# microsoft/SpareNet

Measured on AMD Instinct MI355X. Metric: point-pairs/sec (CD+EMD) + depthmaps/sec, B=32 N=16384, higher is better.
Workload: dtype f32

## Files before the change

### sparenet_amd/csrc/p2i.hip

```cpp
#include <cmath>
#include <cstring>

#include "block_scan.hpp"
#include "common.hpp"
#include "wave_dpp.hpp"

namespace {

__device__ __forceinline__ int clampi(int v, int lo, int hi) {
  return v < lo ? lo : (v > hi ? hi : v);
}

struct Box {
  int min_x, max_x, min_y, max_y;
};
__device__ __forceinline__ Box box_of(float py, float px, int h, int w, float radius) {
  Box b;
  b.min_x = clampi((int)floorf(px - radius), 0, w - 1);
  b.max_x = clampi((int)ceilf(px + radius), 0, w - 1);
  b.min_y = clampi((int)floorf(py - radius), 0, h - 1);
  b.max_y = clampi((int)ceilf(py + radius), 0, h - 1);
  return b;
}

__device__ __forceinline__ float cos_weight_inv(float r, double inv_radius) {
  const double y = ((double)r * inv_radius - 0.5) * M_PI;
  const double y2 = y * y;
  double p = -3.868170170630684e-23;
  p = __builtin_fma(p, y2, 1.9572941063391263e-20);
  p = __builtin_fma(p, y2, -8.22063524662433e-18);
  p = __builtin_fma(p, y2, 2.8114572543455206e-15);
  p = __builtin_fma(p, y2, -7.647163731819816e-13);
  p = __builtin_fma(p, y2, 1.6059043836821613e-10);
  p = __builtin_fma(p, y2, -2.505210838544172e-08);
  p = __builtin_fma(p, y2, 2.7557319223985893e-06);
  p = __builtin_fma(p, y2, -0.0001984126984126984);
  p = __builtin_fma(p, y2, 0.008333333333333333);
  p = __builtin_fma(p, y2, -0.16666666666666666);
  p = __builtin_fma(p, y2, 1.0);
  return (float)(0.5 - 0.5 * (y * p));
}
__device__ __forceinline__ float cos_weight(float r, float radius) {
  return cos_weight_inv(r, 1.0 / (double)radius);
}

__device__ __forceinline__ float sq2(float dx, float dy) {
#pragma clang fp contract(off)
  return dx * dx + dy * dy;
}

__device__ __forceinline__ float radius_of(float dx, float dy) {
#pragma clang fp contract(off)
  return __builtin_sqrtf(dx * dx + dy * dy);
}

__device__ __forceinline__ float one_zero(float v) { return v == 0.f ? 0.f : v; }

__global__ __launch_bounds__(256) void p2i_max_init_kernel(const float *__restrict__ background,
                                                           unsigned long long *__restrict__ img,
                                                           long total) {
  for (long e = (long)blockIdx.x * blockDim.x + threadIdx.x; e < total;
       e += (long)gridDim.x * blockDim.x)
    img[e] = ((unsigned long long)sn::ordered_key(one_zero(background[e])) << 32) | 0xFFFFFFFFull;
}

__device__ __forceinline__ long xcd_point_group(int lpp, int npoints, int channels, int batch) {
  const int gpb = 256 / lpp;
  const long chunk = ((long)npoints + batch - 1) / batch * channels;
  const int bpc = (int)((chunk + gpb - 1) / gpb);
  const int g = blockIdx.x, xcd = g & 7, r = g >> 3;
  const int cidx = (r / bpc) * 8 + xcd;
  if (cidx >= batch) return -1;
  const long local = (long)(r % bpc) * gpb + threadIdx.x / lpp;
  if (local >= chunk) return -1;
  const long gid = (long)cidx * chunk + local;
  return gid < (long)npoints * channels ? gid : -1;
}
inline long xcd_point_blocks(int lpp, int npoints, int channels, int batch) {
  const int gpb = 256 / lpp;
  const long chunk = ((long)npoints + batch - 1) / batch * channels;
  const long bpc = (chunk + gpb - 1) / gpb;
  return bpc * 8 * ((batch + 7) / 8);
}

struct SplatHit {
  unsigned pix;
  float r, f;
  unsigned low;
};

__device__ __forceinline__ float max_sq_inside(float radius) {
#pragma clang fp contract(off)
  float s = radius * radius;
  while (__builtin_sqrtf(s) > radius) s = __uint_as_float(__float_as_uint(s) - 1u);
  for (;;) {
    const float t = __uint_as_float(__float_as_uint(s) + 1u);
    if (!(__builtin_sqrtf(t) <= radius)) break;
    s = t;
  }
  return s;
}

__device__ __forceinline__ void splat_exact(const SplatHit &hh, unsigned long long *img,
                                            float radius) {
  const float v = one_zero(hh.f * cos_weight(__builtin_sqrtf(hh.r), radius));
  atomicMax(img + hh.pix, ((unsigned long long)sn::ordered_key(v) << 32) | hh.low);
}

template <int LPP>
__global__ __launch_bounds__(256) void p2i_max_splat_kernel(
    const float *__restrict__ points, const float *__restrict__ feat,
    const int *__restrict__ batch_inds, unsigned long long *__restrict__ img, int npoints,
    int channels, int batch, int h, int w, float radius) {
  constexpr int kQ = 128;
  __shared__ SplatHit queue[4][kQ];
  const int wave = threadIdx.x >> 6, lane = threadIdx.x & 63;
  SplatHit *q = queue[wave];
  const long gid = xcd_point_group(LPP, npoints, channels, batch);
  const int l = threadIdx.x % LPP;
  bool alive = gid >= 0;
  int x = 0, y = 0, min_y = 0, max_y = -1, max_x = -1;
  float px = 0.f, py = 0.f, f = 0.f;
  unsigned low = 0, plane = 0;
  if (alive) {
    const int c = (int)(gid % channels);
    const int pid = (int)((gid / channels) % npoints);
    const int b = batch_inds[pid];
    if (b < 0 || b >= batch) {
      alive = false;
    } else {
      py = points[pid * 2 + 0];
      px = points[pid * 2 + 1];
      f = feat[gid];
      const Box bx = box_of(py, px, h, w, radius);
      x = bx.min_x + l;
      y = min_y = bx.min_y;
      max_y = bx.max_y;
      max_x = bx.max_x;
      low = 0xFFFFFFFEu - (unsigned)pid;
      plane = (unsigned)(((size_t)b * channels + c) * h * w);
      alive = x <= max_x;
    }
  }
  const float rev_scale = 0.5f / radius;
  const float s_max = max_sq_inside(radius);
  int qn = 0;
  constexpr int kRows = 8;
  while (__any(alive)) {
    float s2[kRows];
    unsigned pix[kRows], cur[kRows];
    bool in[kRows];
    const float dx = x - px;
#pragma unroll
    for (int i = 0; i < kRows; ++i) {
      const int yy = y + i;
      s2[i] = sq2(dx, yy - py);
      in[i] = alive && yy <= max_y && s2[i] <= s_max;
      pix[i] = in[i] ? plane + (unsigned)yy * w + x : plane;
    }
#pragma unroll
    for (int i = 0; i < kRows; ++i)
      cur[i] = (unsigned)(__hip_atomic_load(img + pix[i], __ATOMIC_RELAXED,
                                            __HIP_MEMORY_SCOPE_AGENT) >> 32);
#pragma unroll
    for (int i = 0; i < kRows; ++i) {
      bool pass = false;
      if (in[i]) {
        const float ra = __builtin_amdgcn_sqrtf(s2[i]);
        const float wq = __builtin_amdgcn_cosf(ra * rev_scale) * 0.5f + 0.5f;
        const float ub = f >= 0.f ? f * (wq + 2e-5f) : f * __builtin_fmaxf(wq - 2e-5f, 0.f);
        pass = !(sn::ordered_key(one_zero(ub)) < cur[i]);
      }
      const unsigned long long m = __ballot(pass);
      if (m) {
        if (pass)
          q[qn + __builtin_amdgcn_mbcnt_hi((unsigned)(m >> 32), __builtin_amdgcn_mbcnt_lo((unsigned)m, 0u))] =
              SplatHit{pix[i], s2[i], f, low};
        qn += __popcll(m);
        __builtin_amdgcn_fence(__ATOMIC_RELEASE, "wavefront");
        if (qn >= 64) {
          __builtin_amdgcn_fence(__ATOMIC_ACQUIRE, "wavefront");
          qn -= 64;
          splat_exact(q[qn + lane], img, radius);
          __builtin_amdgcn_fence(__ATOMIC_ACQ_REL, "wavefront");
        }
      }
    }
    if (alive) {
      y += kRows;
      if (y > max_y) {
        y = min_y;
        x += LPP;
        alive = x <= max_x;
      }
    }
  }
  __builtin_amdgcn_fence(__ATOMIC_ACQUIRE, "wavefront");
  if (lane < qn) splat_exact(q[lane], img, radius);
}

constexpr int kCell = 8;
constexpr int kMaxRadii = 4;

struct RadiiArg {
  float radius[kMaxRadii], s_max[kMaxRadii], rev_scale[kMaxRadii], inv_r2[kMaxRadii];
  float s_max_all;
  int halo;
};

__device__ __forceinline__ int cell_of_point(float py, float px, int h, int w, int cells_x,
                                             int cells_y) {
  if (!(__builtin_fabsf(py) < 1e9f) || !(__builtin_fabsf(px) < 1e9f)) return -1;
  const int cy = clampi((int)floorf(py) / kCell, 0, cells_y - 1);
  const int cx = clampi((int)floorf(px) / kCell, 0, cells_x - 1);
  (void)h;
  (void)w;
  return cy * cells_x + cx;
}

__global__ __launch_bounds__(256) void p2i_bin_count_kernel(
    const float *__restrict__ points, const int *__restrict__ batch_inds, int *__restrict__ offs,
    int npoints, int batch, int h, int w, int cells_x, int cells_y, const unsigned *__restrict__ need) {
  if (*need == 0u) return;
  for (int pid = blockIdx.x * blockDim.x + threadIdx.x; pid < npoints;
       pid += gridDim.x * blockDim.x) {
    const int b = batch_inds[pid];
    if (b < 0 || b >= batch) continue;
    const int c = cell_of_point(points[pid * 2 + 0], points[pid * 2 + 1], h, w, cells_x, cells_y);
    if (c >= 0) atomicAdd(&offs[b * cells_y * cells_x + c], 1);
  }
}

__global__ __launch_bounds__(1024) void p2i_bin_scan_kernel(const int *__restrict__ counts,
                                                            int *__restrict__ offs_out,
                                                            int cells_per_image,
                                                            const unsigned *__restrict__ need) {
  __shared__ alignas(16) sn::BlockScan<1024> scan;
  if (*need == 0u) return;
  const int tid = threadIdx.x, b = blockIdx.x;
  int before = 0;
  for (long i = tid; i < (long)b * cells_per_image; i += 1024) before += counts[i];
  for (int m = 1; m < 64; m <<= 1) before += __shfl_xor(before, m);
  if ((tid & 63) == 0) scan.wsum[tid >> 6] = before;
  __syncthreads();
  int t = 0;
  if (tid == 0)
    for (int w = 0; w < 16; ++w) t += scan.wsum[w];
  scan.reset(t);
  const int *c = counts + (size_t)b * cells_per_image;
  int *o = offs_out + (size_t)b * cells_per_image;
  for (int base = 0; base < cells_per_image; base += 1024) {
    const int i = base + tid;
    scan.chunk(i < cells_per_image ? c[i] : 0, [&](int start) {
      if (i < cells_per_image) o[i] = start;
    });
  }
}

__global__ __launch_bounds__(256) void p2i_bin_scatter_kernel(
    const float *__restrict__ points, const float *__restrict__ feat,
    const int *__restrict__ batch_inds, int *__restrict__ offs, float4 *__restrict__ srec,
    unsigned *__restrict__ fmax_bits, int npoints, int channels, int batch, int h, int w, int cells_x,
    int cells_y, const unsigned *__restrict__ need) {
  if (*need == 0u) return;
  float fm = 0.f;
  for (int pid = blockIdx.x * blockDim.x + threadIdx.x; pid < npoints;
       pid += gridDim.x * blockDim.x) {
    const int b = batch_inds[pid];
    if (b < 0 || b >= batch) continue;
    const float py = points[pid * 2 + 0], px = points[pid * 2 + 1];
    const int c = cell_of_point(py, px, h, w, cells_x, cells_y);
    if (c < 0) continue;
    const int pos = atomicAdd(&offs[b * cells_y * cells_x + c], 1);
    srec[pos] = make_float4(py, px, channels == 1 ? feat[pid] : 0.f, __int_as_float(pid));
    for (int ch = 0; ch < channels; ++ch) fm = __builtin_fmaxf(fm, __builtin_fabsf(feat[(size_t)pid * channels + ch]));
  }
  for (int m = 1; m < 64; m <<= 1) fm = __builtin_fmaxf(fm, __shfl_xor(fm, m));
  if ((threadIdx.x & 63) == 0 && __float_as_uint(fm) > *reinterpret_cast<volatile unsigned *>(fmax_bits))
    atomicMax(fmax_bits, __float_as_uint(fm));
}

constexpr int kGroupCells = 8192;
__global__ __launch_bounds__(1024) void p2i_bin_grouped_kernel(
    const float *__restrict__ points, const float *__restrict__ feat,
    const int *__restrict__ batch_inds, int *__restrict__ offs, float4 *__restrict__ srec,
    unsigned *__restrict__ fmax_bits, unsigned *__restrict__ need, int ppi, int channels, int h, int w,
    int cells_x, int cells_y) {
  __shared__ int cnt[kGroupCells];
  __shared__ alignas(16) sn::BlockScan<1024> scan;
  __shared__ int bad;
  const int tid = threadIdx.x, b = blockIdx.x;
  const int cpi = cells_x * cells_y;
  const long base = (long)b * ppi;
  for (int i = tid; i < cpi; i += 1024) cnt[i] = 0;
  if (tid == 0) bad = 0;
  __syncthreads();
  bool wrong = false;
  for (int i = tid; i < ppi; i += 1024) {
    const long pid = base + i;
    const int c = cell_of_point(points[pid * 2 + 0], points[pid * 2 + 1], h, w, cells_x, cells_y);
    wrong |= batch_inds[pid] != b || c < 0;
    if (c >= 0) atomicAdd(&cnt[c], 1);
  }
  if (wrong) bad = 1;
  __syncthreads();
  if (bad) {
    if (tid == 0) atomicOr(need, 1u);
    return;
  }
  scan.reset((int)base);
  for (int c0 = 0; c0 < cpi; c0 += 1024) {
    const int i = c0 + tid;
    scan.chunk(i < cpi ? cnt[i] : 0, [&](int start) {
      if (i < cpi) cnt[i] = start;
    });
  }
  float fm = 0.f;
  for (int i = tid; i < ppi; i += 1024) {
    const long pid = base + i;
    const float py = points[pid * 2 + 0], px = points[pid * 2 + 1];
    const int c = cell_of_point(py, px, h, w, cells_x, cells_y);
    const int pos = atomicAdd(&cnt[c], 1);
    srec[pos] = make_float4(py, px, channels == 1 ? feat[pid] : 0.f, __int_as_float((int)pid));
    for (int ch = 0; ch < channels; ++ch) fm = __builtin_fmaxf(fm, __builtin_fabsf(feat[(size_t)pid * channels + ch]));
  }
  __syncthreads();
  for (int i = tid; i < cpi; i += 1024) offs[(long)b * cpi + i] = cnt[i];
  for (int m = 1; m < 64; m <<= 1) fm = __builtin_fmaxf(fm, __shfl_xor(fm, m));
  if ((tid & 63) == 0 && __float_as_uint(fm) > *reinterpret_cast<volatile unsigned *>(fmax_bits))
    atomicMax(fmax_bits, __float_as_uint(fm));
}

#ifdef SN_P2I_DIAG
__device__ unsigned long long g_gather_diag[8];
#define GDIAG(...) __VA_ARGS__
#else
#define GDIAG(...)
#endif

__device__ __forceinline__ float weight32(float u) {
  float p = __builtin_fmaf(u, -0.0102886269f, 0.114825197f);
  p = __builtin_fmaf(u, p, -0.666184545f);
  p = __builtin_fmaf(u, p, 2.02902055f);
  p = __builtin_fmaf(u, p, -2.46737266f);
  return __builtin_fmaf(u, p, 0.999999583f);
}
constexpr float kWeightErr = 1.5e-6f;
__device__ __forceinline__ float weight32_plus(float u, float e) {
  float p = __builtin_fmaf(u, -0.0102886269f, 0.114825197f);
  p = __builtin_fmaf(u, p, -0.666184545f);
  p = __builtin_fmaf(u, p, 2.02902055f);
  p = __builtin_fmaf(u, p, -2.46737266f);
  return __builtin_fmaf(u, p, 0.999999583f + e);
}

__device__ __forceinline__ float slope32(float u) {
  float p = __builtin_fmaf(u, -0.00193834002f, 0.0257028304f);
  p = __builtin_fmaf(u, p, -0.190524563f);
  p = __builtin_fmaf(u, p, 0.811689675f);
  p = __builtin_fmaf(u, p, -1.64492953f);
  return __builtin_fmaf(u, p, 0.99999994f);
}

__global__ void p2i_series_kernel(const float *__restrict__ u, int n, float *__restrict__ w,
                                  float *__restrict__ sl) {
  const int i = blockIdx.x * blockDim.x + threadIdx.x;
  if (i < n) {
    w[i] = weight32(u[i]);
    sl[i] = slope32(u[i]);
  }
}

template <int NR, bool C1>
__global__ __launch_bounds__(256, 6) void p2i_gather_max_kernel(
    const float *__restrict__ feat, const float *__restrict__ background,
    const float4 *__restrict__ srec, const int *__restrict__ offs, const unsigned *__restrict__ fmax_bits,
    int channels, int batch, int h, int w, int cells_x, int cells_y, RadiiArg ra,
    float *__restrict__ out, int *__restrict__ out_ids, long obstride, long orstride) {
  const int wave = __builtin_amdgcn_readfirstlane((int)(threadIdx.x >> 6)), lane = threadIdx.x & 63;
  long tile = (long)blockIdx.x * 4 + wave;
  const long tiles = (long)batch * channels * cells_y * cells_x;
  if (tile >= tiles) return;
  const int cx = (int)(tile % cells_x); tile /= cells_x;
  const int cy = (int)(tile % cells_y); tile /= cells_y;
  const int c = (int)(tile % channels);
  const int b = (int)(tile / channels);
  const int x = cx * kCell + (lane & 7), y = cy * kCell + (lane >> 3);
  const bool valid = x < w && y < h;
  const unsigned long long valid_mask = __builtin_amdgcn_ballot_w64(valid);
  const size_t plane = ((size_t)b * channels + c) * h * w;
  const float fx = (float)x, fy = (float)y;
  const float eps = __uint_as_float(*fmax_bits) * kWeightErr, band = 2.f * eps;
  constexpr unsigned kBg = 0xFFFFFFFFu;
  const float bg = valid && background ? background[plane + (size_t)y * w + x] : 0.f;
  float b1[NR], b2[NR], b3[NR];
  float low1[NR];
  unsigned j1[NR], j2[NR];
#pragma unroll
  for (int k = 0; k < NR; ++k) {
    b1[k] = bg;
    low1[k] = bg - band;
    j1[k] = kBg;
    b2[k] = b3[k] = -3.0e38f;
    j2[k] = kBg;
  }
  const float tx0 = (float)(cx * kCell), tx1 = tx0 + (kCell - 1), ty0 = (float)(cy * kCell),
              ty1 = ty0 + (kCell - 1);
  float tile_min[NR];
  GDIAG(int dg_batches = 0, dg_cand = 0, dg_surv = 0, dg_pairs = 0, dg_upd = 0, dg_amb = 0, dg_walk = 0, dg_rings = 0;)
  bool dirty[NR];
  auto refresh_tile_min = [&]() {
#pragma unroll
    for (int k = 0; k < NR; ++k) {
      if (!dirty[k]) continue;
      dirty[k] = false;
      tile_min[k] = sn::wave_min_f32(valid ? b1[k] : 3.0e38f);
    }
  };
#pragma unroll
  for (int k = 0; k < NR; ++k) dirty[k] = true;
  refresh_tile_min();

  const int cell_base = b * cells_y * cells_x;
  auto row_range = [&](int step, int part, int &beg, int &end) -> bool {
    const int dyc = (step + 1) >> 1;
    const int cyy = cy + ((step & 1) ? -dyc : dyc);
    if (cyy < 0 || cyy >= cells_y) return false;
    const float gy = (float)((dyc > 1 ? dyc - 1 : 0) * kCell);
    const float rem = ra.s_max_all * 1.0001f - gy * gy;
    if (rem < 0.f) return false;
    int reach = (int)(__builtin_sqrtf(rem) * (1.0f / kCell)) + 1;
    reach = reach < ra.halo ? reach : ra.halo;
    const int c_lo = cx - reach > 0 ? cx - reach : 0;
    const int c_hi = cx + reach < cells_x - 1 ? cx + reach : cells_x - 1;
    const int p_lo = step == 0 ? (part == 0 ? cx : (part == 1 ? c_lo : cx + 1)) : c_lo;
    const int p_hi = step == 0 ? (part == 0 ? cx : (part == 1 ? cx - 1 : c_hi)) : c_hi;
    if (p_lo > p_hi) return false;
    const int first_cell = cell_base + cyy * cells_x + p_lo;
    beg = first_cell > 0 ? offs[first_cell - 1] : 0;
    end = offs[cell_base + cyy * cells_x + p_hi];
    return beg < end;
  };

  auto ring_range = [&](int ring, int rstep, int part, int &beg, int &end) -> bool {
    const int dyc = (rstep + 1) >> 1;
    const int cyy = cy + ((rstep & 1) ? -dyc : dyc);
    if (cyy < 0 || cyy >= cells_y) return false;
    const float gy = (float)((dyc > 1 ? dyc - 1 : 0) * kCell);
    const float rem = ra.s_max_all * 1.0001f - gy * gy;
    if (rem < 0.f) return false;
    int p_lo, p_hi;
    if (dyc == ring) {
      if (part != 0) return false;
      int reach = (int)(__builtin_sqrtf(rem) * (1.0f / kCell)) + 1;
      reach = reach < ring ? reach : ring;
      p_lo = cx - reach > 0 ? cx - reach : 0;
      p_hi = cx + reach < cells_x - 1 ? cx + reach : cells_x - 1;
    } else {
      const float gx = (float)((ring - 1) * kCell);
      if (gx * gx > rem) return false;
      p_lo = p_hi = part == 0 ? cx - ring : cx + ring;
      if (p_lo < 0 || p_lo >= cells_x) return false;
    }
    const int first_cell = cell_base + cyy * cells_x + p_lo;
    beg = first_cell > 0 ? offs[first_cell - 1] : 0;
    end = offs[cell_base + cyy * cells_x + p_hi];
    return beg < end;
  };
  const float fmaxv = __uint_as_float(*fmax_bits);
  for (int ring = 0; ring <= ra.halo; ++ring) {
    if (ring >= 2) {
      const float g = (float)((ring - 1) * kCell);
      const float g2 = g * g * 0.99999f;
      bool live = false;
#pragma unroll
      for (int k = 0; k < NR; ++k) {
        const float ub = fmaxv * weight32_plus(__builtin_fminf(g2 * ra.inv_r2[k], 1.0f), 4e-6f);
        live = live || (g2 <= ra.s_max[k] && tile_min[k] <= ub + band);
      }
      GDIAG(dg_rings += live ? 0 : 1;)
      if (!live) break;
    }
   for (int rstep = 0; rstep <= 2 * ring; ++rstep) {
    for (int part = 0; part < 2; ++part) {
      int beg, end;
      if (!ring_range(ring, rstep, part, beg, end)) continue;
      float4 rec_next = make_float4(0.f, 0.f, 0.f, 0.f);
      if (beg + lane < end) rec_next = srec[beg + lane];
      for (int base = beg; base < end; base += 64) {
        const int j = base + lane;
        const float4 rec = rec_next;
        if (j + 64 < end) rec_next = srec[j + 64];
        float cpy = 0.f, cpx = 0.f, cf = 0.f;
        if (j < end) {
          cpy = rec.x;
          cpx = rec.y;
          cf = C1 ? rec.z : feat[(size_t)__float_as_int(rec.w) * channels + c];
        }
        unsigned long long keep[NR];
        {
          const float ddx = __builtin_fmaxf(__builtin_fmaxf(tx0 - cpx, cpx - tx1), 0.f);
          const float ddy = __builtin_fmaxf(__builtin_fmaxf(ty0 - cpy, cpy - ty1), 0.f);
          const float smin = (ddx * ddx + ddy * ddy) * 0.99999f;
          unsigned long long m_end;
          float cfp;
          asm("v_cmp_lt_i32_e64 %0, %1, %2" : "=s"(m_end) : "v"(j), "s"(end));
          asm("v_max_f32 %0, %1, %2" : "=v"(cfp) : "v"(cf), "v"(0.f));
#pragma unroll
          for (int k = 0; k < NR; ++k) {
            float u;
            asm("v_min_f32 %0, %1, %2" : "=v"(u) : "v"(smin * ra.inv_r2[k]), "v"(1.0f));
            const float ub = cfp * weight32_plus(u, 4e-6f);
            unsigned long long m_r, m_v;
            asm("v_cmp_ge_f32_e64 %0, %1, %2" : "=s"(m_r) : "s"(ra.s_max[k]), "v"(smin));
            asm("v_cmp_le_f32_e64 %0, %1, %2" : "=s"(m_v) : "s"(tile_min[k]), "v"(ub + band));
            keep[k] = m_end & m_r & m_v;
          }
        }
        unsigned long long todo = keep[0];
#pragma unroll
        for (int k = 1; k < NR; ++k) todo |= keep[k];
        GDIAG(dg_batches++; dg_cand += (end - base < 64 ? end - base : 64); dg_surv += __popcll(todo);)
        while (todo) {
          const int i = __builtin_ctzll(todo);
          todo &= todo - 1;
          const float py = __int_as_float(__builtin_amdgcn_readlane(__float_as_int(cpy), i));
          const float px = __int_as_float(__builtin_amdgcn_readlane(__float_as_int(cpx), i));
          const float f = __int_as_float(__builtin_amdgcn_readlane(__float_as_int(cf), i));
          const float dx = fx - px, dy = fy - py;
          const float s2 = sq2(dx, dy);
          const unsigned pos = (unsigned)(base + i);
#pragma unroll
          for (int k = 0; k < NR; ++k) {
            if (!((keep[k] >> i) & 1ull)) continue;
            const float a = f * weight32(s2 * ra.inv_r2[k]);
            unsigned long long m_in, m_ge;
            asm("v_cmp_ge_f32_e64 %0, %1, %2" : "=s"(m_in) : "s"(ra.s_max[k]), "v"(s2));
            asm("v_cmp_ge_f32_e64 %0, %1, %2" : "=s"(m_ge) : "v"(a), "v"(low1[k]));
            const unsigned long long pass = m_in & m_ge & valid_mask;
            GDIAG(dg_pairs += __popcll(m_in & valid_mask); dg_upd += __popcll(pass);)
            if (pass != 0ull) {
              dirty[k] = true;
              float ae, t, t2, n1, n2, n3;
              unsigned long long first, second;
              unsigned posv = pos, e2, nj1, nj2;
              const float far = -__builtin_inff();
              asm("v_cndmask_b32_e64 %0, %1, %2, %3" : "=v"(ae) : "v"(far), "v"(a), "s"(pass));
              asm("v_cmp_gt_f32_e64 %0, %1, %2" : "=s"(first) : "v"(ae), "v"(b1[k]));
              asm("v_cmp_gt_f32_e64 %0, %1, %2" : "=s"(second) : "v"(ae), "v"(b2[k]));
              asm("v_min_f32 %0, %1, %2" : "=v"(t) : "v"(b1[k]), "v"(ae));
              asm("v_max_f32 %0, %1, %2" : "=v"(n1) : "v"(b1[k]), "v"(ae));
              asm("v_min_f32 %0, %1, %2" : "=v"(t2) : "v"(b2[k]), "v"(t));
              asm("v_max_f32 %0, %1, %2" : "=v"(n2) : "v"(b2[k]), "v"(t));
              asm("v_max_f32 %0, %1, %2" : "=v"(n3) : "v"(b3[k]), "v"(t2));
              asm("v_cndmask_b32_e64 %0, %1, %2, %3" : "=v"(e2) : "v"(j2[k]), "v"(posv), "s"(second));
              asm("v_cndmask_b32_e64 %0, %1, %2, %3" : "=v"(nj2) : "v"(e2), "v"(j1[k]), "s"(first));
              asm("v_cndmask_b32_e64 %0, %1, %2, %3" : "=v"(nj1) : "v"(j1[k]), "v"(posv), "s"(first));
              j2[k] = nj2;
              j1[k] = nj1;
              b1[k] = n1;
              b2[k] = n2;
              b3[k] = n3;
              low1[k] = n1 - band;
            }
          }
        }
        refresh_tile_min();
      }
    }
   }
  }

  auto exact_of = [&](unsigned pos, double inv_radius, float s_max, float &v, unsigned &low) {
    const float4 rec = srec[pos];
    const int pid = __float_as_int(rec.w);
    const float f = C1 ? rec.z : feat[(size_t)pid * channels + c];
    const float s2 = sq2(fx - rec.y, fy - rec.x);
    (void)s_max;
    v = f * cos_weight_inv(__builtin_sqrtf(s2), inv_radius);
    low = 0xFFFFFFFEu - (unsigned)pid;
  };
  const size_t oplane = (size_t)b * obstride + (size_t)c * h * w;
#pragma unroll
  for (int k = 0; k < NR; ++k) {
    float best_v = bg;
    unsigned best_low = kBg;
    const double inv_rd = 1.0 / (double)ra.radius[k];
    const bool walk = valid && b3[k] >= b1[k] - band;
    const bool amb = valid && !walk && b2[k] >= b1[k] - band;
    GDIAG(dg_amb += __popcll(__ballot(amb)); dg_walk += __popcll(__ballot(walk));)
    if (valid && !walk) {
      auto consider = [&](unsigned pos) {
        if (pos == kBg) return;
        float v;
        unsigned low;
        exact_of(pos, inv_rd, ra.s_max[k], v, low);
        if (v > best_v || (v == best_v && best_low != kBg && low > best_low)) {
          best_v = v;
          best_low = low;
        }
      };
      consider(j1[k]);
      if (amb) consider(j2[k]);
    }
    if (__any(walk)) {
      for (int step = 0; step <= 2 * ra.halo; ++step) {
        const int nparts = step == 0 ? 3 : 1;
        for (int part = 0; part < nparts; ++part) {
          int beg, end;
          if (!row_range(step, part, beg, end)) continue;
          for (int pos = beg; pos < end; ++pos) {
            const float4 rec = srec[pos];
            const float s2 = sq2(fx - rec.y, fy - rec.x);
            if (walk && s2 <= ra.s_max[k]) {
              const int pid = __float_as_int(rec.w);
              const float f = C1 ? rec.z : feat[(size_t)pid * channels + c];
              const float v = f * cos_weight_inv(__builtin_sqrtf(s2), inv_rd);
              const unsigned low = 0xFFFFFFFEu - (unsigned)pid;
              if (v > best_v || (v == best_v && best_low != kBg && low > best_low)) {
                best_v = v;
                best_low = low;
              }
            }
          }
        }
      }
    }
// ... 196 lines not shown
  if (width <= 48) return 8;
  if (width <= 128) return 16;
  return 64;
}

int check_common(const char *fn, int npoints, int channels, int batch, int h, int w,
                 float radius) {
  if (!(npoints >= 0 && channels >= 1 && batch >= 1 && h >= 1 && w >= 1))
    return sn::fail(SN_EINVAL, "%s: bad sizes npoints=%d channels=%d batch=%d h=%d w=%d", fn,
                    npoints, channels, batch, h, w);
  if (!(radius > 0.f)) return sn::fail(SN_EINVAL, "%s: kernel radius must be > 0", fn);
  if ((long)batch * channels * h * w >= (1L << 31) - 1 || (long)npoints * channels >= (1L << 31))
    return sn::fail(SN_EINVAL, "%s: tensor too large", fn);
  return 0;
}

constexpr int kMaxLinBlocks = 4096;

__device__ __forceinline__ float finite_abs(float x) {
  const float a = __builtin_fabsf(x);
  return a <= 3.40282347e38f ? a : 0.f;
}

__global__ __launch_bounds__(1024) void p2i_absmax_kernel(const float *__restrict__ a, long na,
                                                         const float *__restrict__ b, long nb,
                                                         unsigned *__restrict__ out2) {
  float ma = 0.f, mb = 0.f;
  const long na4 = (reinterpret_cast<size_t>(a) & 15) == 0 ? na / 4 : 0;
  for (long e = (long)blockIdx.x * blockDim.x + threadIdx.x; e < na4; e += (long)gridDim.x * blockDim.x) {
    const float4 v = reinterpret_cast<const float4 *>(a)[e];
    ma = __builtin_fmaxf(__builtin_fmaxf(ma, __builtin_fmaxf(finite_abs(v.x), finite_abs(v.y))),
                         __builtin_fmaxf(finite_abs(v.z), finite_abs(v.w)));
  }
  for (long e = na4 * 4 + (long)blockIdx.x * blockDim.x + threadIdx.x; e < na; e += (long)gridDim.x * blockDim.x)
    ma = __builtin_fmaxf(ma, finite_abs(a[e]));
  for (long e = (long)blockIdx.x * blockDim.x + threadIdx.x; e < nb; e += (long)gridDim.x * blockDim.x)
    mb = __builtin_fmaxf(mb, finite_abs(b[e]));
  for (int m = 1; m < 64; m <<= 1) {
    ma = __builtin_fmaxf(ma, __shfl_xor(ma, m));
    mb = __builtin_fmaxf(mb, __shfl_xor(mb, m));
  }
  __shared__ float red[2][16];
  if ((threadIdx.x & 63) == 0) {
    red[0][threadIdx.x >> 6] = ma;
    red[1][threadIdx.x >> 6] = mb;
  }
  __syncthreads();
  if (threadIdx.x == 0) {
    for (int i = 1; i < (int)(blockDim.x >> 6); ++i) {
      ma = __builtin_fmaxf(ma, red[0][i]);
      mb = __builtin_fmaxf(mb, red[1][i]);
    }
    if (__float_as_uint(ma) > *reinterpret_cast<volatile unsigned *>(out2 + 0)) atomicMax(out2 + 0, __float_as_uint(ma));
    if (__float_as_uint(mb) > *reinterpret_cast<volatile unsigned *>(out2 + 1)) atomicMax(out2 + 1, __float_as_uint(mb));
  }
}

__device__ __forceinline__ double fixed_scale(const unsigned *absmax, float min_radius) {
  const double g = __uint_as_float(absmax[0]), f = __uint_as_float(absmax[1]);
  const double m = g * __builtin_fmax(1.0, f * (1.5707963267948966 / (double)min_radius) * 1.01);
  if (!(m > 0.0)) return 1.0;
  return ldexp(1.0, 43 - ilogb(m));
}

constexpr int kNonFiniteFlag = 2;
constexpr unsigned kClsNaN = 1u, kClsPosInf = 2u, kClsNegInf = 4u;

__device__ __forceinline__ void mark_non_finite(unsigned *cls, unsigned *flag, long e, float v) {
  const unsigned bits = v != v ? kClsNaN : (v > 0.f ? kClsPosInf : kClsNegInf);
  atomicOr(cls + (e >> 2), bits << (8 * (e & 3)));
  atomicOr(flag, 1u);
}

constexpr int kAccSlots = 512;
constexpr int kAccProbes = 8;
constexpr int kAccRegion = 4;

__global__ __launch_bounds__(256) void p2i_max_bwd_accum_kernel(
    const float *__restrict__ out_grad, const int *__restrict__ out_ids,
    const float *__restrict__ points, const float *__restrict__ feat,
    unsigned *__restrict__ absmax, float *__restrict__ background_grad,
    long long *__restrict__ acc_pts, long long *__restrict__ acc_feat, unsigned *__restrict__ cls, long npts2,
    int channels, int batch, int h, int w, RadiiArg ra, int nradii, float min_radius, long obstride, long orstride) {
  __shared__ int keys[kAccSlots];
  __shared__ unsigned long long vals[kAccSlots][3];
  const int cells_x = (w + kCell - 1) / kCell, cells_y = (h + kCell - 1) / kCell;
  const int regs_x = (cells_x + kAccRegion - 1) / kAccRegion, regs_y = (cells_y + kAccRegion - 1) / kAccRegion;
  const int rpi = channels * regs_y * regs_x;
  const int g = blockIdx.x, xcd = g & 7, r = g >> 3;
  const int b = (r / rpi) * 8 + xcd;
  if (b >= batch) return;
  int reg = r % rpi;
  const int rx = reg % regs_x; reg /= regs_x;
  const int ry = reg % regs_y;
  const int c = reg / regs_y;
  const int wave = threadIdx.x >> 6, lane = threadIdx.x & 63;
  const double scale = fixed_scale(absmax, min_radius);
  const size_t plane = ((size_t)b * channels + c) * h * w;
  for (int i = threadIdx.x; i < kAccSlots; i += 256) {
    keys[i] = -1;
    vals[i][0] = vals[i][1] = vals[i][2] = 0ull;
  }
  __syncthreads();
  auto fixed = [&](float x) {
    const double m = 6755399441055744.0;
    return (unsigned long long)(__double_as_longlong(__builtin_fma((double)x, scale, m)) - __double_as_longlong(m));
  };
  for (int ty = 0; ty < kAccRegion; ++ty) {
    for (int tx = wave; tx < kAccRegion; tx += 4) {
      const int cx = rx * kAccRegion + tx, cy = ry * kAccRegion + ty;
      if (cx >= cells_x || cy >= cells_y) continue;
      const int x = cx * kCell + (lane & 7), y = cy * kCell + (lane >> 3);
      const bool valid = x < w && y < h;
      const size_t e = plane + (size_t)(valid ? y : 0) * w + (valid ? x : 0);
      const size_t oe = (size_t)b * obstride + (size_t)c * h * w + (size_t)(valid ? y : 0) * w + (valid ? x : 0);
      float bg = 0.f;
      float gk[kMaxRadii];
      int pidk[kMaxRadii];
#pragma unroll
      for (int k = 0; k < kMaxRadii; ++k) {
        gk[k] = (k < nradii && valid) ? out_grad[(size_t)k * orstride + oe] : 0.f;
        pidk[k] = (k < nradii && valid) ? out_ids[(size_t)k * orstride + oe] : -1;
      }
      int ppid = -1;
      unsigned long long p0 = 0ull, p1 = 0ull, p2 = 0ull;
#pragma unroll
      for (int k = 0; k <= kMaxRadii; ++k) {
        if (k > nradii) break;
        int pid = -1;
        unsigned long long t0 = 0ull, t1 = 0ull, t2 = 0ull;
        if (k < kMaxRadii && k < nradii) {
          pid = pidk[k];
          if (pid < 0) {
            bg += gk[k];
          } else {
            const float2 pp = reinterpret_cast<const float2 *>(points)[pid];
            const float fv = feat[(size_t)pid * channels + c];
            const float dx = x - pp.y, dy = y - pp.x;
            const float u = __builtin_fminf((dx * dx + dy * dy) * ra.inv_r2[k], 1.0f);
            const float cf = gk[k] * weight32(u);
            const float kk = gk[k] * fv * (4.93480220f * ra.inv_r2[k]) * slope32(u);
            const float v1 = kk * dy, v2 = kk * dx;
            if (__builtin_fabsf(cf) <= 3.40282347e38f && __builtin_fabsf(v1) <= 3.40282347e38f &&
                __builtin_fabsf(v2) <= 3.40282347e38f) {
              t0 = fixed(cf);
              t1 = fixed(v1);
              t2 = fixed(v2);
            } else {
              if (__builtin_fabsf(cf) <= 3.40282347e38f) t0 = fixed(cf);
              else mark_non_finite(cls, absmax + kNonFiniteFlag, npts2 + (long)pid * channels + c, cf);
              if (__builtin_fabsf(v1) <= 3.40282347e38f) t1 = fixed(v1);
              else mark_non_finite(cls, absmax + kNonFiniteFlag, (long)pid * 2 + 0, v1);
              if (__builtin_fabsf(v2) <= 3.40282347e38f) t2 = fixed(v2);
              else mark_non_finite(cls, absmax + kNonFiniteFlag, (long)pid * 2 + 1, v2);
            }
          }
        }
        if (pid >= 0 && pid == ppid) {
          p0 += t0;
          p1 += t1;
          p2 += t2;
          continue;
        }
        if (ppid >= 0) {
          unsigned slot = (((unsigned)ppid * 2654435761u) >> 16) & (kAccSlots - 1);
          bool found = false;
          for (int probe = 0; probe < kAccProbes; ++probe) {
            const int prev = atomicCAS(&keys[slot], -1, ppid);
            if (prev == -1 || prev == ppid) {
              found = true;
              break;
            }
            slot = (slot + 1) & (kAccSlots - 1);
          }
          if (found) {
            atomicAdd(&vals[slot][0], p0);
            atomicAdd(&vals[slot][1], p1);
            atomicAdd(&vals[slot][2], p2);
          } else {
            atomicAdd(reinterpret_cast<unsigned long long *>(acc_feat + (size_t)ppid * channels + c), p0);
            atomicAdd(reinterpret_cast<unsigned long long *>(acc_pts + (size_t)ppid * 2 + 0), p1);
            atomicAdd(reinterpret_cast<unsigned long long *>(acc_pts + (size_t)ppid * 2 + 1), p2);
          }
        }
        ppid = pid;
        p0 = t0;
        p1 = t1;
        p2 = t2;
      }
      if (valid && background_grad) background_grad[e] = bg;
    }
  }
  __syncthreads();
  for (int i = threadIdx.x; i < kAccSlots; i += 256) {
    const int id0 = keys[i];
    if (id0 < 0) continue;
    atomicAdd(reinterpret_cast<unsigned long long *>(acc_feat + (size_t)id0 * channels + c), vals[i][0]);
    atomicAdd(reinterpret_cast<unsigned long long *>(acc_pts + (size_t)id0 * 2 + 0), vals[i][1]);
    atomicAdd(reinterpret_cast<unsigned long long *>(acc_pts + (size_t)id0 * 2 + 1), vals[i][2]);
  }
}

__global__ __launch_bounds__(256) void p2i_max_bwd_finish_kernel(
    const long long *__restrict__ acc_pts, const long long *__restrict__ acc_feat,
    const unsigned *__restrict__ absmax, const unsigned *__restrict__ cls, float *__restrict__ points_grad,
    float *__restrict__ feat_grad, long npts2, long nfeat, float min_radius) {
  const double inv = 1.0 / fixed_scale(absmax, min_radius);
  const bool non_finite = absmax[kNonFiniteFlag] != 0u;
  for (long e = (long)blockIdx.x * blockDim.x + threadIdx.x; e < npts2 + nfeat;
       e += (long)gridDim.x * blockDim.x) {
    float v = (float)((double)(e < npts2 ? acc_pts[e] : acc_feat[e - npts2]) * inv);
    if (non_finite) {
      const unsigned bits = (cls[e >> 2] >> (8 * (e & 3))) & 7u;
      if ((bits & kClsNaN) || bits == (kClsPosInf | kClsNegInf)) v = __builtin_nanf("");
      else if (bits) v = bits == kClsPosInf ? __builtin_inff() : -__builtin_inff();
    }
    if (e < npts2)
      points_grad[e] = v;
    else
      feat_grad[e - npts2] = v;
  }
}

unsigned long long *pixel_layout(sn::Carver &c, int batch, int channels, int h, int w) {
  return c.take<unsigned long long>((size_t)batch * channels * h * w * 8);
}
float *pixel_bwd_layout(sn::Carver &c, int batch, int channels, int h, int w) {
  return c.take<float>((size_t)batch * channels * h * w * 12);
}
struct TileWs {
  unsigned *fmax_bits;
  int *counts;
  int *offs;
  float4 *srec;
};
TileWs tile_layout(sn::Carver &c, int npoints, int batch, int h, int w) {
  const size_t cells = (size_t)batch * sn::ceil_div(h, kCell) * sn::ceil_div(w, kCell);
  return {c.take<unsigned>(256), c.take256<int>(cells * 4), c.take256<int>(cells * 4),
          c.take<float4>((size_t)npoints * 16)};
}
struct AccWs {
  unsigned *absmax;
  long long *acc_pts;
  long long *acc_feat;
  unsigned *cls;
};
AccWs acc_layout(sn::Carver &c, int npoints, int channels) {
  return {c.take<unsigned>(256), c.take<long long>((size_t)npoints * 2 * 8),
          c.take<long long>((size_t)npoints * channels * 8),
          c.take<unsigned>(sn::align_up((size_t)npoints * (2 + (size_t)channels), 4))};
}

}

extern "C" size_t sn_p2i_max_workspace_bytes(int batch, int channels, int h, int w) {
  if (batch < 1 || channels < 1 || h < 1 || w < 1) return 0;
  return sn::layout_bytes(pixel_layout, batch, channels, h, w);
}

namespace {

constexpr float kTileMaxRadius = 16.f;

float max_sq_inside_host(float radius) {
  volatile float s = radius * radius;
  auto next = [](float v, int d) {
    unsigned u;
    memcpy(&u, &v, 4);
    u += d;
    memcpy(&v, &u, 4);
    return v;
  };
  while (sqrtf(s) > radius) s = next(s, -1);
  for (;;) {
    const float t = next(s, 1);
    if (!(sqrtf(t) <= radius)) break;
    s = t;
  }
  return s;
}

int tile_forward(const char *fn, const float *points, const float *feat, const int *batch_inds,
                 const float *background, int npoints, int channels, int batch, int h, int w,
                 const float *radii, int nradii, int image_major, float *out, int *out_ids, void *workspace,
                 hipStream_t s) {
  RadiiArg ra = {};
  float rmax = 0.f;
  for (int k = 0; k < nradii; ++k) {
    ra.radius[k] = radii[k];
    ra.s_max[k] = max_sq_inside_host(radii[k]);
    ra.rev_scale[k] = 0.5f / radii[k];
    ra.inv_r2[k] = 1.0f / (radii[k] * radii[k]);
    ra.s_max_all = ra.s_max[k] > ra.s_max_all ? ra.s_max[k] : ra.s_max_all;
    rmax = radii[k] > rmax ? radii[k] : rmax;
  }
  ra.halo = (int)floorf(rmax / kCell) + 1;
  const int cells_x = sn::ceil_div(w, kCell), cells_y = sn::ceil_div(h, kCell);
  const long cells = (long)batch * cells_x * cells_y;
  const long tiles = cells * channels;
  SN_REQUIRE(tiles / 4 + 1 < (1L << 31), "%s: too many tiles", fn);
  sn::Carver carver(workspace);
  const TileWs t = tile_layout(carver, npoints, batch, h, w);
  unsigned *const need = t.fmax_bits + 1;
  const bool try_grouped = npoints > 0 && npoints % batch == 0 && cells_x * cells_y <= kGroupCells;
  if (try_grouped) {
    SN_HIP(hipMemsetAsync(t.fmax_bits, 0, 8, s));
    p2i_bin_grouped_kernel<<<batch, 1024, 0, s>>>(points, feat, batch_inds, t.offs, t.srec, t.fmax_bits, need,
                                                  npoints / batch, channels, h, w, cells_x, cells_y);
  } else {
    SN_HIP(hipMemsetAsync(t.fmax_bits, 0, 4, s));
    SN_HIP(hipMemsetD32Async(reinterpret_cast<hipDeviceptr_t>(need), 1, 1, s));
  }
  SN_HIP(hipMemsetAsync(t.counts, 0, (size_t)cells * 4, s));
  if (npoints > 0)
    p2i_bin_count_kernel<<<sn::grid_blocks(npoints, kMaxLinBlocks), 256, 0, s>>>(
        points, batch_inds, t.counts, npoints, batch, h, w, cells_x, cells_y, need);
  p2i_bin_scan_kernel<<<batch, 1024, 0, s>>>(t.counts, t.offs, cells_x * cells_y, need);
  if (npoints > 0)
    p2i_bin_scatter_kernel<<<sn::grid_blocks(npoints, kMaxLinBlocks), 256, 0, s>>>(
        points, feat, batch_inds, t.offs, t.srec, t.fmax_bits, npoints, channels, batch, h, w, cells_x, cells_y, need);
  const int blocks = (int)((tiles + 3) / 4);
  const long chw = (long)channels * h * w;
  const long obstride = image_major ? (long)nradii * chw : chw, orstride = image_major ? chw : (long)batch * chw;
#define SN_GATHER(NR)                                                                         \
  do {                                                                                        \
    if (channels == 1)                                                                        \
      p2i_gather_max_kernel<NR, true><<<blocks, 256, 0, s>>>(feat, background, t.srec, t.offs,   \
          t.fmax_bits, channels, batch, h, w, cells_x, cells_y, ra, out, out_ids, obstride, orstride); \
    else                                                                                      \
      p2i_gather_max_kernel<NR, false><<<blocks, 256, 0, s>>>(feat, background, t.srec, t.offs,  \
          t.fmax_bits, channels, batch, h, w, cells_x, cells_y, ra, out, out_ids, obstride, orstride); \
  } while (0)
  if (sn::prof_enabled()) sn::prof_begin("p2i_max_splat", s);
  switch (nradii) {
    case 1: SN_GATHER(1); break;
    case 2: SN_GATHER(2); break;
    case 3: SN_GATHER(3); break;
    default: SN_GATHER(4); break;
  }
  if (sn::prof_enabled()) sn::prof_end("p2i_max_splat", s);
#undef SN_GATHER
  return sn::launch_status(fn);
}

}

#ifdef SN_P2I_DIAG
extern "C" int sn_p2i_gather_diag(unsigned long long *out8, int reset) {
  if (hipMemcpyFromSymbol(out8, HIP_SYMBOL(g_gather_diag), 64) != hipSuccess) return 1;
  if (reset) {
    unsigned long long z[8] = {0};
    if (hipMemcpyToSymbol(HIP_SYMBOL(g_gather_diag), z, 64) != hipSuccess) return 1;
  }
  return 0;
}
#endif

extern "C" int sn_p2i_series(const float *u, int n, float *weight, float *slope, void *stream) {
  SN_REQUIRE(u && weight && slope && n >= 0, "sn_p2i_series: bad arguments");
  if (n > 0) p2i_series_kernel<<<(n + 255) / 256, 256, 0, sn::as_stream(stream)>>>(u, n, weight, slope);
  return sn::launch_status("sn_p2i_series");
}

extern "C" size_t sn_p2i_max_multi_workspace_bytes(int npoints, int batch, int channels, int h,
                                                   int w) {
  if (npoints < 0 || batch < 1 || channels < 1 || h < 1 || w < 1) return 0;
  const size_t a = sn_p2i_max_workspace_bytes(batch, channels, h, w);
  const size_t t = sn::layout_bytes(tile_layout, npoints, batch, h, w);
  return a > t ? a : t;
}

extern "C" int sn_p2i_max_forward(const float *points, const float *feat, const int *batch_inds,
                                  const float *background, int npoints, int channels, int batch,
                                  int h, int w, float radius, float *out, int *out_ids,
                                  void *workspace, size_t workspace_bytes, void *stream) {
  SN_REQUIRE(background && out && out_ids && workspace, "sn_p2i_max_forward: null pointer");
  SN_REQUIRE(npoints == 0 || (points && feat && batch_inds), "sn_p2i_max_forward: null pointer");
  if (int rc = check_common("sn_p2i_max_forward", npoints, channels, batch, h, w, radius)) return rc;
  sn::Carver carver(workspace);
  unsigned long long *img = pixel_layout(carver, batch, channels, h, w);
  SN_REQUIRE(workspace_bytes >= carver.bytes(), "sn_p2i_max_forward: workspace too small");
  hipStream_t s = sn::as_stream(stream);
  if (radius <= kTileMaxRadius && workspace_bytes >= sn::layout_bytes(tile_layout, npoints, batch, h, w))
    return tile_forward("sn_p2i_max_forward", points, feat, batch_inds, background, npoints,
                        channels, batch, h, w, &radius, 1, 0, out, out_ids, workspace, s);
  const long px = (long)batch * channels * h * w;
  p2i_max_init_kernel<<<sn::grid_blocks(px, kMaxLinBlocks), 256, 0, s>>>(background, img, px);
  const long groups = (long)npoints * channels;
  if (groups > 0) {
    const int lpp = lanes_per_point(radius);
    const long blocks = xcd_point_blocks(lpp, npoints, channels, batch);
    SN_REQUIRE(blocks < (1L << 31), "sn_p2i_max_forward: too many points");
#define SN_SPLAT(L)                                                                          \
  p2i_max_splat_kernel<L><<<(int)blocks, 256, 0, s>>>(points, feat, batch_inds, img, npoints, \
                                                      channels, batch, h, w, radius)
    if (sn::prof_enabled()) sn::prof_begin("p2i_max_splat", s);
    switch (lpp) {
      case 4: SN_SPLAT(4); break;
      case 8: SN_SPLAT(8); break;
      case 16: SN_SPLAT(16); break;
      case 32: SN_SPLAT(32); break;
      default: SN_SPLAT(64); break;
    }
    if (sn::prof_enabled()) sn::prof_end("p2i_max_splat", s);
#undef SN_SPLAT
  }
  p2i_max_finalize_kernel<<<sn::grid_blocks(px, kMaxLinBlocks), 256, 0, s>>>(img, background, out, out_ids, px);
  return sn::launch_status("sn_p2i_max_forward");
}

extern "C" int sn_p2i_max_forward_multi(const float *points, const float *feat,
                                        const int *batch_inds, const float *background,
                                        int npoints, int channels, int batch, int h, int w,
                                        const float *radii, int nradii, int image_major, float *out,
                                        int *out_ids, void *workspace, size_t workspace_bytes,
                                        void *stream) {
  SN_REQUIRE(out && out_ids && workspace && radii, "sn_p2i_max_forward_multi: null pointer");
  SN_REQUIRE(npoints == 0 || (points && feat && batch_inds), "sn_p2i_max_forward_multi: null pointer");
  SN_REQUIRE(nradii >= 1 && nradii <= kMaxRadii, "sn_p2i_max_forward_multi: 1..%d radii (got %d)",
             kMaxRadii, nradii);
  float rmax = 0.f;
  for (int k = 0; k < nradii; ++k) {
    if (int rc = check_common("sn_p2i_max_forward_multi", npoints, channels, batch, h, w, radii[k]))
      return rc;
    rmax = radii[k] > rmax ? radii[k] : rmax;
  }
  SN_REQUIRE(workspace_bytes >= sn_p2i_max_multi_workspace_bytes(npoints, batch, channels, h, w),
             "sn_p2i_max_forward_multi: workspace too small");
  hipStream_t s = sn::as_stream(stream);
  if (rmax <= kTileMaxRadius)
    return tile_forward("sn_p2i_max_forward_multi", points, feat, batch_inds, background, npoints,
                        channels, batch, h, w, radii, nradii, image_major, out, out_ids, workspace, s);
  SN_REQUIRE(!image_major || nradii == 1,
             "sn_p2i_max_forward_multi: the image-major layout needs radii <= %g px", (double)kTileMaxRadius);
  SN_REQUIRE(background, "sn_p2i_max_forward_multi: a null (all-zero) background needs radii <= %g px",
             (double)kTileMaxRadius);
  const size_t image = (size_t)batch * channels * h * w;
  for (int k = 0; k < nradii; ++k)
    if (int rc = sn_p2i_max_forward(points, feat, batch_inds, background, npoints, channels, batch,
                                    h, w, radii[k], out + k * image, out_ids + k * image,
                                    workspace, workspace_bytes, stream))
      return rc;
  return 0;
}

extern "C" size_t sn_p2i_max_backward_workspace_bytes(int batch, int channels, int h, int w) {
  if (batch < 1 || channels < 1 || h < 1 || w < 1) return 0;
  return sn::layout_bytes(pixel_bwd_layout, batch, channels, h, w);
}

extern "C" int sn_p2i_max_backward(const float *out_grad, const int *out_ids, const float *points,
                                   const float *feat, const int *batch_inds, int npoints,
                                   int channels, int batch, int h, int w, float radius,
                                   float *points_grad, float *feat_grad, float *background_grad,
                                   void *workspace, size_t workspace_bytes, void *stream) {
  SN_REQUIRE(out_grad && out_ids && background_grad && workspace, "sn_p2i_max_backward: null pointer");
  SN_REQUIRE(npoints == 0 || (points && feat && points_grad && feat_grad),
             "sn_p2i_max_backward: null pointer");
  if (int rc = check_common("sn_p2i_max_backward", npoints, channels, batch, h, w, radius)) return rc;
  sn::Carver carver(workspace);
  float *contrib = pixel_bwd_layout(carver, batch, channels, h, w);
  SN_REQUIRE(workspace_bytes >= carver.bytes(), "sn_p2i_max_backward: workspace too small");
  hipStream_t s = sn::as_stream(stream);
  const long px = (long)batch * channels * h * w;
  p2i_max_bwd_pixels_kernel<<<sn::grid_blocks(px, kMaxLinBlocks), 256, 0, s>>>(out_grad, out_ids, points, feat,
                                                           background_grad, contrib, channels, h, w,
                                                           radius, px);
  if (npoints > 0) {
    const int lpp = lanes_per_point_gather(radius);
    const long blocks = xcd_point_blocks(lpp, npoints, 1, batch);
#define SN_BWD(L)                                                                            \
  p2i_max_bwd_points_kernel<L><<<(int)blocks, 256, 0, s>>>(out_ids, contrib, points, batch_inds, \
      points_grad, feat_grad, npoints, channels, batch, h, w, radius, px)
    switch (lpp) {
      case 4: SN_BWD(4); break;
      case 8: SN_BWD(8); break;
      case 16: SN_BWD(16); break;
      default: SN_BWD(64); break;
    }
#undef SN_BWD
  }
  return sn::launch_status("sn_p2i_max_backward");
}

extern "C" size_t sn_p2i_max_backward_multi_workspace_bytes(int npoints, int channels) {
  if (npoints < 0 || channels < 1) return 0;
  return sn::layout_bytes(acc_layout, npoints, channels);
}

extern "C" int sn_p2i_max_backward_multi(const float *out_grad, const int *out_ids,
                                         const float *points, const float *feat, int npoints,
                                         int channels, int batch, int h, int w, const float *radii,
                                         int nradii, int image_major, float *points_grad,
                                         float *feat_grad, float *background_grad, void *workspace,
                                         size_t workspace_bytes, void *stream) {
  SN_REQUIRE(out_grad && out_ids && workspace && radii, "sn_p2i_max_backward_multi: null pointer");
  SN_REQUIRE(npoints == 0 || (points && feat && points_grad && feat_grad),
             "sn_p2i_max_backward_multi: null pointer");
  SN_REQUIRE(nradii >= 1 && nradii <= kMaxRadii, "sn_p2i_max_backward_multi: 1..%d radii (got %d)",
             kMaxRadii, nradii);
  RadiiArg ra = {};
  float rmin = 3e38f;
  for (int k = 0; k < nradii; ++k) {
    if (int rc = check_common("sn_p2i_max_backward_multi", npoints, channels, batch, h, w, radii[k]))
      return rc;
    ra.radius[k] = radii[k];
    ra.inv_r2[k] = 1.0f / (radii[k] * radii[k]);
    rmin = radii[k] < rmin ? radii[k] : rmin;
  }
  sn::Carver carver(workspace);
  const AccWs a = acc_layout(carver, npoints, channels);
  SN_REQUIRE(workspace_bytes >= carver.bytes(), "sn_p2i_max_backward_multi: workspace too small");
  hipStream_t s = sn::as_stream(stream);
  const long px = (long)batch * channels * h * w;
  SN_HIP(hipMemsetAsync(workspace, 0, carver.bytes(), s));
  p2i_absmax_kernel<<<512, 1024, 0, s>>>(out_grad, px * nradii, feat,
                                                           (long)npoints * channels, a.absmax);
  const long per_image = (long)channels * sn::ceil_div(sn::ceil_div(h, kCell), kAccRegion) *
                         sn::ceil_div(sn::ceil_div(w, kCell), kAccRegion);
  const long blocks = per_image * 8 * ((batch + 7) / 8);
  SN_REQUIRE(blocks < (1L << 31), "sn_p2i_max_backward_multi: image too large");
  p2i_max_bwd_accum_kernel<<<(int)blocks, 256, 0, s>>>(out_grad, out_ids, points, feat, a.absmax,
                                                       background_grad, a.acc_pts, a.acc_feat, a.cls,
                                                       (long)npoints * 2, channels, batch, h, w, ra, nradii, rmin,
                                                       image_major ? (long)nradii * channels * h * w : (long)channels * h * w,
                                                       image_major ? (long)channels * h * w : px);
  if (npoints > 0)
    p2i_max_bwd_finish_kernel<<<sn::grid_blocks((long)npoints * (2 + channels), kMaxLinBlocks), 256, 0, s>>>(
        a.acc_pts, a.acc_feat, a.absmax, a.cls, points_grad, feat_grad, (long)npoints * 2,
        (long)npoints * channels, rmin);
  return sn::launch_status("sn_p2i_max_backward_multi");
}

extern "C" int sn_p2i_sum_forward(const float *points, const float *feat, const int *batch_inds,
                                  int npoints, int channels, int batch, int h, int w, float radius,
                                  float *out, void *stream) {
  SN_REQUIRE(out, "sn_p2i_sum_forward: null pointer");
  SN_REQUIRE(npoints == 0 || (points && feat && batch_inds), "sn_p2i_sum_forward: null pointer");
  if (int rc = check_common("sn_p2i_sum_forward", npoints, channels, batch, h, w, radius)) return rc;
  const long groups = (long)npoints * channels;
  if (groups == 0) return 0;
  hipStream_t s = sn::as_stream(stream);
  const int lpp = lanes_per_point(radius);
  const long blocks = (groups * lpp + 255) / 256;
  SN_REQUIRE(blocks < (1L << 31), "sn_p2i_sum_forward: too many points");
#define SN_SUM(L)                                                                            \
  p2i_sum_fwd_kernel<L><<<(int)blocks, 256, 0, s>>>(points, feat, batch_inds, out, npoints,   \
                                                    channels, batch, h, w, radius)
  switch (lpp) {
    case 4: SN_SUM(4); break;
    case 8: SN_SUM(8); break;
    case 16: SN_SUM(16); break;
    case 32: SN_SUM(32); break;
    default: SN_SUM(64); break;
  }
#undef SN_SUM
  return sn::launch_status("sn_p2i_sum_forward");
}

extern "C" int sn_p2i_sum_backward(const float *out_grad, const float *points, const float *feat,
                                   const int *batch_inds, int npoints, int channels, int batch,
                                   int h, int w, float radius, float *points_grad,
                                   float *feat_grad, void *stream) {
  SN_REQUIRE(out_grad, "sn_p2i_sum_backward: null pointer");
  SN_REQUIRE(npoints == 0 || (points && feat && batch_inds && points_grad && feat_grad),
             "sn_p2i_sum_backward: null pointer");
  if (int rc = check_common("sn_p2i_sum_backward", npoints, channels, batch, h, w, radius)) return rc;
  const long groups = (long)npoints * channels;
  if (groups == 0) return 0;
  hipStream_t s = sn::as_stream(stream);
  if (channels > 1) SN_HIP(hipMemsetAsync(points_grad, 0, (size_t)npoints * 2 * 4, s));
  p2i_sum_bwd_kernel<<<(int)((groups + 255) / 256), 256, 0, s>>>(
      out_grad, points, feat, batch_inds, points_grad, feat_grad, npoints, channels, batch, h, w,
      radius);
  return sn::launch_status("sn_p2i_sum_backward");
}
```

Baseline: 13040 billion.

## Hold grouped-bin points in registers across count and scatter passes

The grouped binning kernel now loads up to 8 points per thread into registers once, using scalar-base loads with per-lane offsets, and reuses them for both the counting and scatter passes instead of reading points from global memory twice. It is templated on single-channel features so the feature value is loaded once alongside the points. It also zeroes the fallback counts buffer inside the kernel instead of issuing a separate memset on the grouped path. The cost is higher register pressure from the held arrays, more complex slot/tail indexing, and a new 8-byte alignment requirement on points for the grouped path.

```diff
diff --git a/sparenet_amd/csrc/p2i.hip b/sparenet_amd/csrc/p2i.hip
--- a/sparenet_amd/csrc/p2i.hip
+++ b/sparenet_amd/csrc/p2i.hip
@@ -280,27 +280,82 @@
     atomicMax(fmax_bits, __float_as_uint(fm));
 }
 
+template <class T>
+__device__ __forceinline__ T load_uniform_plus(const T *uniform, unsigned bytes) {
+#if defined(__HIP_DEVICE_COMPILE__)
+  typedef const __attribute__((address_space(1))) char *GlobalBytes;
+  GlobalBytes u = (GlobalBytes) reinterpret_cast<const char *>(uniform);
+  asm("" : "+s"(u));
+  return *(const __attribute__((address_space(1))) T *)(u + bytes);
+#else
+  return *reinterpret_cast<const T *>(reinterpret_cast<const char *>(uniform) + bytes);
+#endif
+}
 constexpr int kGroupCells = 8192;
-__global__ __launch_bounds__(1024) void p2i_bin_grouped_kernel(
+constexpr int kGroupHold = 8;
+constexpr int kGroupRegPoints = kGroupHold * 1024;
+template <bool C1>
+__global__ __launch_bounds__(1024, 8) void p2i_bin_grouped_kernel(
     const float *__restrict__ points, const float *__restrict__ feat,
-    const int *__restrict__ batch_inds, int *__restrict__ offs, float4 *__restrict__ srec,
-    unsigned *__restrict__ fmax_bits, unsigned *__restrict__ need, int ppi, int channels, int h, int w,
-    int cells_x, int cells_y) {
+    const int *__restrict__ batch_inds, int *__restrict__ counts, int *__restrict__ offs,
+    float4 *__restrict__ srec, unsigned *__restrict__ fmax_bits, unsigned *__restrict__ need, int ppi,
+    int channels, int h, int w, int cells_x, int cells_y) {
   __shared__ int cnt[kGroupCells];
   __shared__ alignas(16) sn::BlockScan<1024> scan;
   __shared__ int bad;
   const int tid = threadIdx.x, b = blockIdx.x;
   const int cpi = cells_x * cells_y;
   const long base = (long)b * ppi;
-  for (int i = tid; i < cpi; i += 1024) cnt[i] = 0;
+  const float2 *const ipts = reinterpret_cast<const float2 *>(points) + base;
+  const int *const ibatch = batch_inds + base;
+  const float *const ifeat = feat + base;
+  const int npass = (ppi + kGroupRegPoints - 1) / kGroupRegPoints;
+  int p0, n;
+  unsigned t;
+  auto set_pass = [&](int p) {
+    p0 = p * kGroupRegPoints;
+    n = ppi - p0 < kGroupRegPoints ? ppi - p0 : kGroupRegPoints;
+    t = (unsigned)(tid < n - 1 ? tid : n - 1);
+  };
+  auto slot_start = [&](int j) { return (j + 1) * 1024 <= n ? j * 1024 : (j * 1024 < n && n > 1024 ? n - 1024 : 0); };
+  auto slot_used = [&](int j) { return j * 1024 < n && (unsigned)tid == t && slot_start(j) + (int)t >= j * 1024; };
+  float2 xy[kGroupHold];
+  int bi[kGroupHold];
+  float f[kGroupHold];
+  auto load_points = [&]() {
+#pragma unroll
+    for (int j = 0; j < kGroupHold; ++j) xy[j] = load_uniform_plus(ipts + p0 + slot_start(j), t * 8u);
+  };
+  auto load_batch_inds = [&]() {
+#pragma unroll
+    for (int j = 0; j < kGroupHold; ++j) bi[j] = load_uniform_plus(ibatch + p0 + slot_start(j), t * 4u);
+  };
+  auto load_features = [&]() {
+#pragma unroll
+    for (int j = 0; j < kGroupHold; ++j) f[j] = C1 ? load_uniform_plus(ifeat + p0 + slot_start(j), t * 4u) : 0.f;
+  };
+  set_pass(0);
+  load_points();
+  load_batch_inds();
+  for (int i = tid; i < cpi; i += 1024) {
+    cnt[i] = 0;
+    counts[(long)b * cpi + i] = 0;
+  }
   if (tid == 0) bad = 0;
   __syncthreads();
   bool wrong = false;
-  for (int i = tid; i < ppi; i += 1024) {
-    const long pid = base + i;
-    const int c = cell_of_point(points[pid * 2 + 0], points[pid * 2 + 1], h, w, cells_x, cells_y);
-    wrong |= batch_inds[pid] != b || c < 0;
-    if (c >= 0) atomicAdd(&cnt[c], 1);
+  for (int p = 0; p < npass; ++p) {
+    if (p > 0) {
+      set_pass(p);
+      load_points();
+      load_batch_inds();
+    }
+#pragma unroll
+    for (int j = 0; j < kGroupHold; ++j) {
+      const int c = cell_of_point(xy[j].x, xy[j].y, h, w, cells_x, cells_y);
+      wrong |= bi[j] != b || c < 0;
+      if (slot_used(j) && c >= 0) atomicAdd(&cnt[c], 1);
+    }
   }
   if (wrong) bad = 1;
   __syncthreads();
@@ -308,6 +363,7 @@
     if (tid == 0) atomicOr(need, 1u);
     return;
   }
+  load_features();
   scan.reset((int)base);
   for (int c0 = 0; c0 < cpi; c0 += 1024) {
     const int i = c0 + tid;
@@ -316,13 +372,29 @@
     });
   }
   float fm = 0.f;
-  for (int i = tid; i < ppi; i += 1024) {
-    const long pid = base + i;
-    const float py = points[pid * 2 + 0], px = points[pid * 2 + 1];
-    const int c = cell_of_point(py, px, h, w, cells_x, cells_y);
-    const int pos = atomicAdd(&cnt[c], 1);
-    srec[pos] = make_float4(py, px, channels == 1 ? feat[pid] : 0.f, __int_as_float((int)pid));
-    for (int ch = 0; ch < channels; ++ch) fm = __builtin_fmaxf(fm, __builtin_fabsf(feat[(size_t)pid * channels + ch]));
+  for (int p = npass - 1; p >= 0; --p) {
+    if (p < npass - 1) {
+      set_pass(p);
+      load_features();
+      load_points();
+    }
+#pragma unroll
+    for (int j = 0; j < kGroupHold; ++j) {
+      if (slot_used(j)) {
+        const int c = cell_of_point(xy[j].x, xy[j].y, h, w, cells_x, cells_y);
+        const int pos = atomicAdd(&cnt[c], 1);
+        srec[pos] = make_float4(xy[j].x, xy[j].y, f[j], __int_as_float((int)base + p0 + slot_start(j) + (int)t));
+      }
+      fm = __builtin_fmaxf(fm, __builtin_fabsf(f[j]));
+    }
+    if (!C1) {
+      for (int ch = 0; ch < channels; ++ch) {
+#pragma unroll
+        for (int j = 0; j < kGroupHold; ++j) f[j] = feat[(size_t)(base + p0 + slot_start(j) + t) * channels + ch];
+#pragma unroll
+        for (int j = 0; j < kGroupHold; ++j) fm = __builtin_fmaxf(fm, __builtin_fabsf(f[j]));
+      }
+    }
   }
   __syncthreads();
   for (int i = tid; i < cpi; i += 1024) offs[(long)b * cpi + i] = cnt[i];
@@ -1125,16 +1197,21 @@
   sn::Carver carver(workspace);
   const TileWs t = tile_layout(carver, npoints, batch, h, w);
   unsigned *const need = t.fmax_bits + 1;
-  const bool try_grouped = npoints > 0 && npoints % batch == 0 && cells_x * cells_y <= kGroupCells;
+  const bool try_grouped = npoints > 0 && npoints % batch == 0 && cells_x * cells_y <= kGroupCells &&
+                           reinterpret_cast<uintptr_t>(points) % 8 == 0;
   if (try_grouped) {
     SN_HIP(hipMemsetAsync(t.fmax_bits, 0, 8, s));
-    p2i_bin_grouped_kernel<<<batch, 1024, 0, s>>>(points, feat, batch_inds, t.offs, t.srec, t.fmax_bits, need,
-                                                  npoints / batch, channels, h, w, cells_x, cells_y);
+    if (channels == 1)
+      p2i_bin_grouped_kernel<true><<<batch, 1024, 0, s>>>(points, feat, batch_inds, t.counts, t.offs, t.srec,
+                                                          t.fmax_bits, need, npoints / batch, channels, h, w, cells_x, cells_y);
+    else
+      p2i_bin_grouped_kernel<false><<<batch, 1024, 0, s>>>(points, feat, batch_inds, t.counts, t.offs, t.srec,
+                                                           t.fmax_bits, need, npoints / batch, channels, h, w, cells_x, cells_y);
   } else {
     SN_HIP(hipMemsetAsync(t.fmax_bits, 0, 4, s));
     SN_HIP(hipMemsetD32Async(reinterpret_cast<hipDeviceptr_t>(need), 1, 1, s));
-  }
-  SN_HIP(hipMemsetAsync(t.counts, 0, (size_t)cells * 4, s));
+    SN_HIP(hipMemsetAsync(t.counts, 0, (size_t)cells * 4, s));
+  }
   if (npoints > 0)
     p2i_bin_count_kernel<<<sn::grid_blocks(npoints, kMaxLinBlocks), 256, 0, s>>>(
         points, batch_inds, t.counts, npoints, batch, h, w, cells_x, cells_y, need);
```

Result: no change. 13100 billion, median of 6 (+0.4%).
